# zgspose/PAVENet

Hardware: AMD Instinct MI355X
Metric: clips/sec (T=7, 800x1344) fwd (higher is better)
Workload: dtype f32 (exact 3-term bf16 split on the bf16 MFMA)

## Files before the change

### include/pave_hip.h

```cpp
#ifndef PAVE_HIP_H_
#define PAVE_HIP_H_

#include <stdint.h>

#ifdef __cplusplus
extern "C" {
#endif

#define PAVE_OK 0
#define PAVE_E_ARG (-1)
#define PAVE_E_LAUNCH (-2)
#define PAVE_E_STEP (-3)
#define PAVE_E_UNSUPPORTED (-4)

#define PAVE_ABI_VERSION 21
int pave_abi_version(void);
const char* pave_last_error(void);

int pave_ms_deform_attn_forward_f32(const float* value, const int64_t* spatial_shapes,
                                    const int64_t* level_start, const float* sampling_loc,
                                    const float* attn_weight, float* out, int bs, int S, int M,
                                    int D, int L, int Lq, int P, int im2col_step, void* stream);
int pave_ms_deform_attn_forward_f64(const double* value, const int64_t* spatial_shapes,
                                    const int64_t* level_start, const double* sampling_loc,
// ... 342 lines not shown
typedef struct pave_reid_plan {
  pave_reid_describe_plan d;
  const int32_t* ids[PAVE_TRACK_MAX_FRAMES];
  int32_t*       out_ids[PAVE_TRACK_MAX_FRAMES];
  int32_t*       out_sim[PAVE_TRACK_MAX_FRAMES];
  int            camera[PAVE_TRACK_MAX_FRAMES];
  int32_t* person;
  int32_t* track;
  int32_t* last;
  int32_t* hits;
  int32_t* hist;
  int32_t* frame;
  int32_t* next;
  int32_t* dropped;
  int32_t* pairs;
  int cameras, S, max_lost, match_thr, min_hits, gain;
} pave_reid_plan;
int pave_reid_describe_nv12(const pave_reid_describe_plan* plan, void* stream);
int pave_reid_describe_bgr(const pave_reid_describe_plan* plan, void* stream);
int pave_reid_update_nv12(const pave_reid_plan* plan, void* stream);
int pave_reid_update_bgr(const pave_reid_plan* plan, void* stream);

int pave_conv3x3_nhwc_f32(const float* x, const float* w, const float* bias, float* y, int N,
                          int H, int W, int Cin, int Cout, int stride, int relu, void* stream);

int pave_rows_gemm_bias_res_act_f32(const float* a, const float* a_bias, const float* a2,
                                    const float* w, const float* bias, const float* residual,
                                    float* out, long long M, int K, int K2, int N, int relu,
                                    void* stream);

int pave_bias_relu_maxpool_nhwc_f32(const float* x, const float* bias, float* y, int N, int H,
                                    int W, int C, void* stream);

#define PAVE_PLANES_FP16 16
int pave_gemm_bf16x3_f32(const float* a, const float* a_bias, const void* w_planes,
                         const float* bias, const float* residual, float* out, long long M, int K,
                         int N, int relu, int nplanes, void* stream);

int pave_gemm_fp16_act_f32(const void* a, int a_is_f16, const void* w_plane, const float* bias,
                           const float* residual, const float* gamma, const float* beta, float eps, void* out,
                           int out_is_f16, long long M, int K, int N, int relu, void* stream);

int pave_gemm_bf16x3_ex_f32(const float* a, const float* a_bias, const void* w_planes,
                            const float* bias, const float* residual, long long residual_rows,
                            float* out, float* out2, int n_split, long long M, int K, int N,
                            int relu, int nplanes, void* stream);

int pave_ref_update_f32(const float* tmp, const float* ref, float* out, long long n, float eps,
                        void* stream);

int pave_groupnorm_nhwc_f32(const float* x, const float* gamma, const float* beta, float* y,
                            long long y_batch_stride, int N, int HW, int C, int G, float eps,
                            double* partial, int nchunks, float* ab, void* stream);

typedef struct pave_gn_level {
  const float* x;
  const float* gamma;
  const float* beta;
  float* y;
  long long y_batch_stride;
  int HW;
  int nchunks;
  float eps;
} pave_gn_level;
int pave_groupnorm_levels_nhwc_f32(const pave_gn_level* levels, int nlev, int N, int C, int G, double* partial,
                                   float* ab, void* stream);
// ... 26 lines not shown
                                long long workspace_bytes, void* stream);

int pave_set_form_policy(int policy);
int pave_get_form_policy(void);

#define PAVE_FORM_ROWS 0
#define PAVE_FORM_ROWS_SPLITK 1
#define PAVE_FORM_ROWS_TILE 2
#define PAVE_FORM_LN 3
#define PAVE_FORM_CONV3X3 4
#define PAVE_FORM_CONV1X1S 5
#define PAVE_FORM_ENCPROJ 6
#define PAVE_ORDER_TILE 0
#define PAVE_ORDER_KSPLIT 1
#define PAVE_ORDER_SPLITK 2
#define PAVE_ORDER_TILE_LNPASS 3
#define PAVE_ORDER_KSPLIT_LNPASS 4
#define PAVE_ORDER_TILE_LN8 5
int pave_form_plan(long long M, int K, int N, int kind, int nplanes, int policy, int* order, int* ksplit);

int pave_bottleneck_chain_f32(const float* c1, const void* w2_planes, const float* b2, float* c2,
                              const void* w3_planes, const float* b3, const float* residual,
                              const float* a2, int k2, float* out, const void* w1n_planes,
                              const float* b1n, float* c1n, int cn, int N, int H, int W, int nplanes,
                              void* stream);

int pave_conv1x1_strided_split_f32(const float* x, const void* w_planes, const float* bias, float* y,
                                   int N, int H, int W, int Cin, int Cout, int stride, int relu,
                                   int nplanes, void* stream);

int pave_conv7x7s2_nchw_split_f32(const float* x, const void* w_planes, const float* bias, float* y,
                                  int N, int H, int W, int row_pitch, int Cout, int relu, int nplanes,
                                  void* stream);

int pave_repitch_rows_f32(const float* src, float* dst, long long rows, int W, int pitch, void* stream);

int pave_swin_window_attn_f32(const float* qkv, const float* bias_t, const float* pad_qkv, float* out, int B,
                              int H, int W, int C, int heads, int window, int shift, float scale, void* stream);

int pave_merge_softmax_partials_f32(const float* parts, float* out, int G, int U, int C, int H, void* stream);

int pave_split_bf16x3_f32(const float* x, void* planes, long long n, int nplanes, void* stream);

#define PAVE_AUG_MAX_AUGS 16
#define PAVE_AUG_MAX_SLOTS 128
#define PAVE_AUG_MAX_K 64
typedef struct pave_aug_plan {
  const float* bboxes[PAVE_AUG_MAX_AUGS];
  const float* kpts[PAVE_AUG_MAX_AUGS];
  const int32_t* keep[PAVE_AUG_MAX_AUGS];
  int32_t flip[PAVE_AUG_MAX_AUGS];
  float img_w[PAVE_AUG_MAX_SLOTS];
  float scale_factor[PAVE_AUG_MAX_SLOTS][4];
  int32_t flip_perm[PAVE_AUG_MAX_K];
  int32_t n_aug, B, N, K;
} pave_aug_plan;
int pave_aug_merge_nms_f32(const pave_aug_plan* plan, float score_thr, int max_num, int method, float iou_thr,
                           float sigma, float min_score, int offset, float* dets, int64_t* labels, float* kpts,
                           int64_t* inds, int32_t* keep, int32_t* count, void* stream);

int pave_hflip_canvas_f32(const float* x, float* y, const int32_t* valid_w, int valid_w_all, int n, int C, int Hp,
                          int Wp, void* stream);

#ifdef __cplusplus
}
#endif
// ... 2 lines not shown
```

### pavenet_amd/backbones.py

```python
import torch
import torch.nn as nn
import torch.nn.functional as F

from .bricks import BaseModule, build_norm_layer
from .registry import MMDET_MODELS


class BasicBlock(nn.Module):
    expansion = 1

    def __init__(self, inplanes, planes, stride=1, dilation=1, downsample=None, style='pytorch',
                 norm_cfg=dict(type='BN')):
        super().__init__()
        self.conv1 = nn.Conv2d(inplanes, planes, 3, stride, dilation, dilation, bias=False)
        self.bn1 = build_norm_layer(norm_cfg, planes)[1]
        self.conv2 = nn.Conv2d(planes, planes, 3, 1, 1, bias=False)
        self.bn2 = build_norm_layer(norm_cfg, planes)[1]
        self.relu = nn.ReLU(inplace=True)
        self.downsample = downsample
        self.pairs = (('conv1', 'bn1', True), ('conv2', 'bn2', False))


class Bottleneck(nn.Module):
    expansion = 4
# ... 50 lines not shown
        self.norm_eval = norm_eval
        self.style = style
        block, stage_blocks = self.arch_settings[depth]
        stage_blocks = stage_blocks[:num_stages]
        self.conv1 = nn.Conv2d(in_channels, stem_channels, 7, 2, 3, bias=False)
        self.bn1 = build_norm_layer(norm_cfg, stem_channels)[1]
        self.relu = nn.ReLU(inplace=True)
        self.maxpool = nn.MaxPool2d(kernel_size=3, stride=2, padding=1)
        self.res_layers = []
        inplanes = stem_channels
        for i, nb in enumerate(stage_blocks):
            planes = base_channels * 2**i
            layers = []
            for b in range(nb):
                stride = strides[i] if b == 0 else 1
                downsample = None
                if b == 0 and (stride != 1 or inplanes != planes * block.expansion):
                    downsample = nn.Sequential(
                        nn.Conv2d(inplanes, planes * block.expansion, 1, stride, bias=False),
                        build_norm_layer(norm_cfg, planes * block.expansion)[1])
                layers.append(block(inplanes, planes, stride, dilations[i], downsample, style,
                                    norm_cfg))
                inplanes = planes * block.expansion
            name = f'layer{i + 1}'
            self.add_module(name, nn.Sequential(*layers))
            self.res_layers.append(name)
        self.feat_dim = inplanes
        self._folded = None
        self.channels_last = True
        self.fused_tail_max_k = 256
        self.fused_ds_max_k = 128
        self.chain_stage64 = True
        self.chain_mode = 'full'
        self.deterministic_conv3x3 = False

    def init_weights(self):
        for m in self.modules():
            if isinstance(m, nn.Conv2d):
                nn.init.kaiming_normal_(m.weight, mode='fan_out', nonlinearity='relu')
            elif isinstance(m, (nn.BatchNorm2d, nn.GroupNorm)):
                nn.init.constant_(m.weight, 1)
                nn.init.constant_(m.bias, 0)
        for m in self.modules():
            if isinstance(m, Bottleneck):
                nn.init.constant_(m.bn3.weight, 0)
            elif isinstance(m, BasicBlock):
                nn.init.constant_(m.bn2.weight, 0)
        self._is_init = True

    def _params_key(self):
        from .bricks import SourceKey, module_tensors
        return SourceKey(module_tensors(self))

    def _stem_folded(self):
        from .bricks import SourceKey
        bn = self.bn1
        key = SourceKey([self.conv1.weight, bn.weight, bn.bias, bn.running_mean, bn.running_var])
        hit = self.__dict__.get('_stem_cache')
        if hit is None or hit[0] != key:
            mf = torch.channels_last if self.channels_last else torch.contiguous_format
            with torch.no_grad():
                hit = (key, tuple(t.contiguous(memory_format=mf) if t.dim() == 4 else t
                                  for t in _fold(self.conv1, self.bn1)))
            self.__dict__['_stem_cache'] = hit
        return hit[1]

    def _build_folded(self):
        key = self._params_key()
        if self._folded is not None and self._folded[0] == key:
            return self._folded[1]
        mf = torch.channels_last if self.channels_last else torch.contiguous_format
        with torch.no_grad():
            f = {'stem': tuple(t.contiguous(memory_format=mf) if t.dim() == 4 else t
                               for t in _fold(self.conv1, self.bn1))}
            for name in self.res_layers:
                for bi, blk in enumerate(getattr(self, name)):
                    for cn, bn, _ in blk.pairs:
                        w, b = _fold(getattr(blk, cn), getattr(blk, bn))
                        f[(name, bi, cn)] = (w.contiguous(memory_format=mf), b)
                        if cn == 'conv2' and w.shape[2:] == (3, 3) and w.shape[1] % 32 == 0 \
                                and w.shape[0] % 64 == 0:
                            f[(name, bi, 'conv2_taps')] = w.permute(2, 3, 1, 0).contiguous()
                        if cn == 'conv3' and w.shape[1] <= self.fused_tail_max_k \
                                and w.shape[1] % 32 == 0:
                            f[(name, bi, 'conv3_kn')] = w.flatten(1).t().contiguous()
                    if blk.downsample is not None:
                        w, b = _fold(blk.downsample[0], blk.downsample[1])
                        f[(name, bi, 'ds')] = (w.contiguous(memory_format=mf), b)
                        w3_kn = f.get((name, bi, 'conv3_kn'))
                        if w3_kn is not None and w.shape[1] % 32 == 0 and \
                                w3_kn.shape[0] + w.shape[1] <= self.fused_ds_max_k:
                            f[(name, bi, 'tail_ds_kn')] = (
                                torch.cat([w3_kn, w.flatten(1).t()], 0).contiguous(),
                                f[(name, bi, 'conv3')][1] + b)
        self._folded = (key, f)
        return f

    @staticmethod
    def _stem_split(x_nchw, w):
        from . import ops
        from .bricks import _split_cached, fused_mode, get_gemm_mode
        if not fused_mode() or torch.is_grad_enabled() or not x_nchw.is_cuda \
                or x_nchw.dtype != torch.float32 or tuple(w.shape) != (64, 3, 7, 7) \
                or x_nchw.shape[1] != 3 or x_nchw.shape[3] < 8 or not x_nchw.is_contiguous():
            return None
        wp = _split_cached(w, 'stem7x7', lambda planes: ops.split_stem7x7_weight(w.detach(), planes))
        if x_nchw.shape[3] % 4 or x_nchw.data_ptr() % 16:
            return ops.conv7x7s2_nchw_split(ops.repitch_rows(x_nchw), wp, valid_w=x_nchw.shape[3])
        return ops.conv7x7s2_nchw_split(x_nchw, wp)

    @staticmethod
    def _ds_bias(f, name, bi):
        key = (name, bi, 'ds_b3')
        if key not in f:
            f[key] = f[(name, bi, 'ds')][1] + f[(name, bi, 'conv3')][1]
        return f[key]

    @staticmethod
    def _as_rows(x):
        n, c, h, w = x.shape
        return x.permute(0, 2, 3, 1).reshape(-1, c), (n, h, w)

    @staticmethod
    def _as_map(rows, nhw):
        n, h, w = nhw
        return rows.view(n, h, w, rows.shape[-1]).permute(0, 3, 1, 2)

    def _stage64_chain_ok(self, name, x, f):
        from .bricks import _GEMM, fused_mode
        blocks = list(getattr(self, name))
        if blocks[0].downsample is not None and (name, 0, 'tail_ds_kn') not in f:
            return False
        if not (self.chain_stage64 and fused_mode() and not torch.is_grad_enabled()
                and x.is_contiguous(memory_format=torch.channels_last)
                and x.shape[0] * x.shape[2] * x.shape[3] >= _GEMM['min_rows']
                and all(isinstance(b, Bottleneck) for b in blocks)):
            return False
        for bi, blk in enumerate(blocks):
            c1, c2, c3 = blk.conv1, blk.conv2, blk.conv3
            if not (c1.out_channels == 64 and c1.stride == (1, 1)
                    and tuple(c2.weight.shape) == (64, 64, 3, 3) and c2.stride == (1, 1)
                    and c2.dilation == (1, 1) and c2.padding == (1, 1) and c2.groups == 1
# ... 122 lines not shown
                                      inplace_residual=True, a_bias=b2)
                else:
                    out = ops.rows_gemm_bias_res_act(yrows, w3_kn, None, idt, relu=True, out=idt,
                                                     a_bias=b2)
            else:
                idt = torch.addmm(bd + b3, xrows, wd.flatten(1).t())
                if w3_kn is not None:
                    out = ops.rows_gemm_bias_res_act(yrows, w3_kn, None, idt, relu=True, out=idt,
                                                     a_bias=b2)
                else:
                    out = torch.addmm(idt, yrows, w3.flatten(1).t())
                    ops.bias_act_rows_(out, None, None, relu=True)
        elif split3:
            out = linear_rows(yrows, w3.flatten(1), b3, relu=True, residual=rows,
                              inplace_residual=inplace_identity, a_bias=b2)
        elif w3_kn is not None:
            out = ops.rows_gemm_bias_res_act(yrows, w3_kn, b3, rows, relu=True,
                                             out=rows if inplace_identity else None, a_bias=b2)
        elif inplace_identity:
            out = rows.addmm_(yrows, w3.flatten(1).t())
            ops.bias_act_rows_(out, b3, None, relu=True)
        else:
            out = torch.addmm(rows, yrows, w3.flatten(1).t())
            ops.bias_act_rows_(out, b3, None, relu=True)
        return self._as_map(out, onhw)

    def forward(self, x):
        if self.input_type == 'mul_frames' and x.dim() == 5:
            x = x.flatten(0, 1)
        assert not self.training, 'pavenet_amd.ResNet is an inference (frozen BN) backbone'
        gemm_path = (self.channels_last and x.is_cuda and x.dtype == torch.float32
                     and self.style == 'pytorch')
        w, b = self._stem_folded()
        y = self._stem_split(x, w) if gemm_path else None
        if y is None and self.channels_last:
            x = x.contiguous(memory_format=torch.channels_last)
        if gemm_path:
            from . import ops
            if y is None:
                y = F.conv2d(x, w, None, 2, 3)
            x = ops.bias_relu_maxpool_nhwc(y, b)
        else:
            x = self.maxpool(F.relu_(F.conv2d(x, w, b, 2, 3)))
        f = self._build_folded()
        outs = []
        pre_c1 = None
        for i, name in enumerate(self.res_layers):
            if gemm_path and self._stage64_chain_ok(name, x, f):
                nxt = None
                if i + 1 < len(self.res_layers):
                    nb = getattr(self, self.res_layers[i + 1])[0]
                    if isinstance(nb, Bottleneck) and nb.conv1.stride == (1, 1) and \
                            nb.conv1.in_channels == 256 and nb.conv1.out_channels in (64, 128):
                        nxt = f[(self.res_layers[i + 1], 0, 'conv1')]
                x, pre_c1 = self._stage64_chain(name, x, f, nxt)
                if i in self.out_indices:
                    outs.append(x)
                continue
            for bi, blk in enumerate(getattr(self, name)):
                if gemm_path and isinstance(blk, Bottleneck):
                    x = self._bottleneck_gemm(blk, x, f, name, bi, inplace_identity=bi > 0,
                                              c1=pre_c1)
                    pre_c1 = None
                    continue
                identity = x
                y = x
                for cn, _, act in blk.pairs:
                    conv = getattr(blk, cn)
                    w, b = f[(name, bi, cn)]
                    y = F.conv2d(y, w, b, conv.stride, conv.padding, conv.dilation)
# ... 347 lines not shown
```

### pavenet_amd/csrc/pave_gemm_dma.hip

```cpp
#include <hip/hip_runtime.h>
#include <type_traits>
#include <stdint.h>

#include "pave_hip.h"
#include "pave_internal.h"
#include "pave_enc_math.h"

namespace {

typedef __bf16 bf16x8 __attribute__((ext_vector_type(8)));
typedef float f32x16 __attribute__((ext_vector_type(16)));
typedef unsigned u32x4 __attribute__((ext_vector_type(4)));
typedef float f32x4 __attribute__((ext_vector_type(4)));

constexpr int QBM = 128;
constexpr int QNS = 3;
constexpr int QCST = 36;

struct QConv {
  int H, W, Cin, Ho, Wo, stride;
  unsigned rcp;
};
struct QOut {
  float* out2;
// ... 1011 lines not shown
}

template <int PL>
__global__ __launch_bounds__(512) __attribute__((amdgpu_waves_per_eu(2, 2))) void gemm_q_ln_kernel(
    const float* __restrict__ A, const uint16_t* __restrict__ Wp, const float* __restrict__ bias,
    const float* residual, float* out, const int M, const int K, const int N, const QLn ln) {
  PAVE_CLOCK_BEGIN(5);
  gemm_q_body<4, 2, 0, false, true, false, 0, 1, PL>(A, Wp, bias, residual, out, M, K, N, 0, nullptr,
                                                     QConv{0, 0, 0, 0, 0, 0}, QOut{nullptr, 0, 0, N, 0}, ln);
  PAVE_CLOCK_END();
}

template <int PL, int IO = 0>
__global__ __launch_bounds__(256) __attribute__((amdgpu_waves_per_eu(2, 2))) void gemm_w_ln_kernel(
    const float* __restrict__ A, const uint16_t* __restrict__ Wp, const float* __restrict__ bias,
    const float* residual, float* out, const int M, const int K, const int N, const QLn ln) {
  PAVE_CLOCK_BEGIN(6);
  gemm_q_body<8, 1, 0, false, true, true, 0, 1, PL, false, IO>(A, Wp, bias, residual, out, M, K, N, 0, nullptr,
                                                               QConv{0, 0, 0, 0, 0, 0}, QOut{nullptr, 0, 0, N, 0}, ln);
  PAVE_CLOCK_END();
}

constexpr int SBM = 96;
constexpr int SWC = 50;
constexpr int SNSLAB = 11;

template <int R>
struct StemRows {
  static constexpr int WPC = 2 * R + 5;
  static constexpr int ROWS = 3 * WPC + 1;
  static constexpr int WIN = ((ROWS * SWC + 63) / 64) * 1024;
};

template <int R, int PL = 3>
__global__ __launch_bounds__(192) void stem7x7_qr_kernel(
    const float* __restrict__ x, const uint16_t* __restrict__ Wp, const float* __restrict__ bias,
    float* __restrict__ y, const int H, const int W, const int Ho, const int Wo, const int relu) {
  extern __shared__ __attribute__((aligned(1024))) unsigned char smem[];
  PAVE_CLOCK_BEGIN(7);
  const int tid = threadIdx.x, lane = tid & 63;
  const int wave = __builtin_amdgcn_readfirstlane(tid >> 6);
  const int lr = lane & 31, kh = lane >> 5;
  const int segs = (Wo + SBM - 1) / SBM;
  constexpr int WPC = StemRows<R>::WPC, ZROW = 3 * WPC;
  const int Hp = (Ho + R - 1) / R;
  const int seg = blockIdx.x % segs;
  const int oy = R * ((blockIdx.x / segs) % Hp);
  const int n = blockIdx.x / (segs * Hp);
  const int ox0 = seg * SBM;
  const int xs = 2 * ox0 - 4;
  const unsigned lds0 = (unsigned)(size_t)(__attribute__((address_space(3))) unsigned char*)smem;

  constexpr int NCH = StemRows<R>::ROWS * SWC;
  constexpr int NINS = StemRows<R>::WIN / 1024;
#pragma unroll
  for (int q = 0; q < (NINS + 2) / 3; ++q) {
    const int ins = wave + 3 * q;
    if (ins < NINS) {
      const int ci = ins * 64 + lane;
      const int row = ci / SWC, cc = ci - row * SWC;
      const int c = row / WPC, wy = row - WPC * c;
      const int iy = 2 * oy - 3 + wy, ix = xs + 4 * cc;
      const bool ok = ci < NCH && row < ZROW && iy >= 0 && iy < H && ix >= 0 && ix + 4 <= W;
      const float* src = ok ? x + (((long long)n * 3 + c) * H + iy) * W + ix
                            : reinterpret_cast<const float*>(g_zero_chunk);
      dma16_flat(src, lds0 + ins * 1024);
    }
  }
  const uint16_t* wl = Wp + ((long long)lr * 16 + kh * 8);
  u32x4 wf[2][PL][2];
// ... 28 lines not shown
#pragma unroll
    for (int j = 0; j < 2; ++j)
#pragma unroll
      for (int i = 0; i < 16; ++i) acc[r][j][i] = 0.f;
  asm volatile("s_waitcnt vmcnt(0)\n\ts_barrier" ::: "memory");
#pragma unroll
  for (int s = 0; s < SNSLAB; ++s) {
    const int cur = s & 1, nxt = cur ^ 1;
    if (s + 1 < SNSLAB) load_w(s + 1, nxt);
#pragma unroll
    for (int r = 0; r < R; ++r) {
      read_split(s, r);
      if constexpr (PL == 1) {
#pragma unroll
        for (int j = 0; j < 2; ++j)
          acc[r][j] = __builtin_amdgcn_mfma_f32_32x32x16_f16(
              __builtin_bit_cast(f16x8, apl[r][0]), __builtin_bit_cast(f16x8, wf[cur][0][j]), acc[r][j], 0, 0, 0);
      } else {
#pragma unroll
      for (int o = 2; o >= 0; --o)
#pragma unroll
        for (int pa = 0; pa <= o; ++pa)
#pragma unroll
          for (int j = 0; j < 2; ++j)
            acc[r][j] = __builtin_amdgcn_mfma_f32_32x32x16_bf16(
                __builtin_bit_cast(bf16x8, apl[r][pa]), __builtin_bit_cast(bf16x8, wf[cur][o - pa][j]),
                acc[r][j], 0, 0, 0);
      }
    }
  }
  asm volatile("s_waitcnt lgkmcnt(0)\n\ts_barrier" ::: "memory");
  float* Cs = reinterpret_cast<float*>(smem) + wave * 32 * QCST;
  const int erow = lane >> 3, ec4 = lane & 7;
#pragma unroll
  for (int r = 0; r < R; ++r) {
    float* const orow = y + ((long long)n * Ho + oy + r) * Wo * 64;
#pragma unroll
    for (int j = 0; j < 2; ++j) {
      const int col = j * 32 + ec4 * 4;
      const float4 b4 = bias ? *reinterpret_cast<const float4*>(bias + col) : make_float4(0.f, 0.f, 0.f, 0.f);
#pragma unroll
      for (int i = 0; i < 16; ++i) Cs[((i & 3) + 8 * (i >> 2) + 4 * kh) * QCST + lr] = acc[r][j][i];
      __builtin_amdgcn_fence(__ATOMIC_RELEASE, "wavefront");
      __builtin_amdgcn_wave_barrier();
      __builtin_amdgcn_fence(__ATOMIC_ACQUIRE, "wavefront");
#pragma unroll
      for (int ps = 0; ps < 4; ++ps) {
        const int lrow = ps * 8 + erow;
        const int ox = ox0 + wave * 32 + lrow;
        float4 v = *reinterpret_cast<const float4*>(Cs + lrow * QCST + ec4 * 4);
        v.x += b4.x, v.y += b4.y, v.z += b4.z, v.w += b4.w;
        if (relu) {
          v.x = fmaxf(v.x, 0.f), v.y = fmaxf(v.y, 0.f), v.z = fmaxf(v.z, 0.f), v.w = fmaxf(v.w, 0.f);
        }
        if (ox < Wo && oy + r < Ho) *reinterpret_cast<float4*>(orow + (long long)ox * 64 + col) = v;
      }
      __builtin_amdgcn_fence(__ATOMIC_RELEASE, "wavefront");
      __builtin_amdgcn_wave_barrier();
    }
  }
  PAVE_CLOCK_END();
}

template <int TN, int KIND, bool ABIAS, int RM = 1, int PL = 3, bool HT = false>
int launch_q(const float* a, const uint16_t* w, const float* bias, const float* residual, float* out,
             long long M, int K, int N, int relu, const float* a_bias, hipStream_t st, const QConv g,
// ... 784 lines not shown
             ? PAVE_OK : PAVE_E_LAUNCH;
}
extern "C" int pave_diag_clock_read(unsigned long long* out16) {
  if (!out16) return PAVE_E_ARG;
  if (hipDeviceSynchronize() != hipSuccess) return PAVE_E_LAUNCH;
  return hipMemcpyFromSymbol(out16, HIP_SYMBOL(g_clock_acc), 16 * sizeof(unsigned long long)) == hipSuccess
             ? PAVE_OK : PAVE_E_LAUNCH;
}
#endif

extern "C" int pave_bottleneck_chain_f32(const float* c1, const void* w2_planes, const float* b2, float* c2,
                                         const void* w3_planes, const float* b3, const float* residual,
                                         const float* a2, int k2, float* out, const void* w1n_planes,
                                         const float* b1n, float* c1n, int cn, int N, int H, int W,
                                         int nplanes, void* stream) {
  return pave_with_planes(q_planes(nplanes), "bottleneck_chain: nplanes must be 3 or PAVE_PLANES_FP16", [&](auto pl) {
    return bottleneck_chain_go<decltype(pl)::value>(c1, w2_planes, b2, c2, w3_planes, b3, residual, a2, k2, out,
                                                    w1n_planes, b1n, c1n, cn, N, H, W, stream);
  });
}

int pave_internal_stem7x7_q(const float* x, const void* w_stem, const float* bias, float* y, int N,
                            int H, int W, int pitch, int relu, void* stream, int planes) {
  const int Ho = (H - 1) / 2 + 1, Wo = (W - 1) / 2 + 1;
  const long long gx = (long long)N * Ho * ((Wo + SBM - 1) / SBM);
  if (gx >= (1ll << 31)) return pave_internal_fail(PAVE_E_ARG, "stem7x7: grid too large");
#ifndef PAVE_STEM_ROWS
#define PAVE_STEM_ROWS 2
#endif
  constexpr int R = PAVE_STEM_ROWS;
  const long long g2 = (long long)N * ((Ho + R - 1) / R) * ((Wo + SBM - 1) / SBM);
  hipStream_t st = reinterpret_cast<hipStream_t>(stream);
  const uint16_t* w = static_cast<const uint16_t*>(w_stem);
  if (planes == 1)
    return pave_launch<stem7x7_qr_kernel<R, 1>>(dim3((unsigned)g2), dim3(192), StemRows<R>::WIN, st, x, w, bias, y, H,
                                                pitch, Ho, Wo, relu);
  return pave_launch<stem7x7_qr_kernel<R, 3>>(dim3((unsigned)g2), dim3(192), StemRows<R>::WIN, st, x, w, bias, y, H,
                                              pitch, Ho, Wo, relu);
}
```

### pavenet_amd/csrc/pave_gemm_split.hip

```cpp
#include <hip/hip_runtime.h>
#include <stdint.h>

#include "pave_hip.h"
#include "pave_internal.h"

namespace {

typedef __bf16 bf16x8 __attribute__((ext_vector_type(8)));
typedef float f32x16 __attribute__((ext_vector_type(16)));
typedef unsigned u32x4 __attribute__((ext_vector_type(4)));
typedef float f32x4 __attribute__((ext_vector_type(4)));
typedef float f32x4_u __attribute__((ext_vector_type(4), aligned(4)));

constexpr int BK = 16;
constexpr int RST = 48;

__device__ __forceinline__ int stage_row_perm(int r) {
  return (r & ~7) | ((r & 3) << 1) | ((r >> 2) & 1);
}

__device__ __forceinline__ unsigned hi16(float x) { return __float_as_uint(x) & 0xffff0000u; }
__device__ __forceinline__ unsigned pack_hi(unsigned lo, unsigned hi) {
  return __builtin_amdgcn_perm(hi, lo, 0x07060302u);
}
// ... 750 lines not shown
  if (rc != PAVE_OK) return rc;
  return pave_internal_splitk_reduce(ws, parts, M, Cout, bias, residual, relu, y, stream);
}

int pave_conv1x1_strided_split_f32(const float* x, const void* w_planes, const float* bias, float* y,
                                   int N, int H, int W, int Cin, int Cout, int stride, int relu,
                                   int nplanes, void* stream) {
  if (!x || !w_planes || !y) return pave_internal_fail(PAVE_E_ARG, "conv1x1_strided_split: null pointer");
  if (N <= 0 || H <= 0 || W <= 0 || stride < 1 || stride > 4)
    return pave_internal_fail(PAVE_E_ARG, "conv1x1_strided_split: bad sizes (1 <= stride <= 4)");
  if (Cin % 64 != 0 || Cout % 128 != 0 || Cin <= 0 || Cout <= 0)
    return pave_internal_fail(PAVE_E_ARG, "conv1x1_strided_split: Cin %% 64 == 0 and Cout %% 128 == 0 required");
  const int Ho = (H - 1) / stride + 1, Wo = (W - 1) / stride + 1;
  const long long M = (long long)N * Ho * Wo;
  if (M >= (1ll << 31) || (long long)N * H * W * Cin >= (1ll << 40))
    return pave_internal_fail(PAVE_E_ARG, "conv1x1_strided_split: tensor too large");
  if (!q_planes(nplanes)) return pave_internal_fail(PAVE_E_ARG, "conv1x1_strided_split: nplanes must be 3 or PAVE_PLANES_FP16");
  if ((g_diag_variant != PAVE_DV_FIRST_GEN || nplanes != 3) && (long long)N * H * W * Cin * 4 < (1ll << 32)) {
    GemmQ q = gemm_q_call(x, w_planes, bias, nullptr, y, M, Cin, Cout, relu, nplanes, stream);
    q.rows = GEMMQ_CONV1X1S, q.H = H, q.W = W, q.Cin = Cin, q.Ho = Ho, q.Wo = Wo, q.stride = stride;
    return pave_internal_gemm_q(q);
  }
  if (nplanes != 3) return pave_internal_fail(PAVE_E_UNSUPPORTED, "conv1x1_strided_split: fp16 operands need a map below 4 GiB");
  const ConvGeom g{H, W, Cin, Ho, Wo, stride};
  return launch_gemm<2, 2, false, 3, false, 0, true>(x, static_cast<const uint16_t*>(w_planes), bias,
                                                     nullptr, y, M, Cin, Cout, relu, nullptr,
                                                     reinterpret_cast<hipStream_t>(stream), g);
}

int pave_conv7x7s2_nchw_split_f32(const float* x, const void* w_planes, const float* bias, float* y,
                                  int N, int H, int W, int row_pitch, int Cout, int relu, int nplanes,
                                  void* stream) {
  if (!x || !w_planes || !y) return pave_internal_fail(PAVE_E_ARG, "conv7x7s2_nchw_split: null pointer");
  if (N <= 0 || H <= 0 || W < 8 || (relu != 0 && relu != 1))
    return pave_internal_fail(PAVE_E_ARG, "conv7x7s2_nchw_split: bad sizes (W >= 8; relu 0 | 1)");
  if (row_pitch == 0) row_pitch = W;
  if (row_pitch < W || (row_pitch != W && ((row_pitch & 3) || (reinterpret_cast<uintptr_t>(x) & 15))))
    return pave_internal_fail(PAVE_E_ARG, "conv7x7s2_nchw_split: row_pitch >= W; a pitch beyond W must be a "
                                          "multiple of 4 on a 16-byte aligned image (pave_repitch_rows_f32)");
  if (Cout != 64)
    return pave_internal_fail(PAVE_E_UNSUPPORTED, "conv7x7s2_nchw_split: Cout == 64 (the ResNet / HRNet stem)");
  const int Ho = (H - 1) / 2 + 1, Wo = (W - 1) / 2 + 1;
  const long long M = (long long)N * Ho * Wo;
  if (M >= (1ll << 31) || (long long)N * 3 * H * row_pitch >= (1ll << 40))
    return pave_internal_fail(PAVE_E_ARG, "conv7x7s2_nchw_split: tensor too large");
  if (!q_planes(nplanes)) return pave_internal_fail(PAVE_E_ARG, "conv7x7s2_nchw_split: nplanes must be 3 or PAVE_PLANES_FP16");
  if ((g_diag_variant != PAVE_DV_FIRST_GEN || nplanes != 3 || row_pitch != W) && row_pitch % 4 == 0 &&
      (reinterpret_cast<uintptr_t>(x) & 15) == 0)
    return pave_internal_stem7x7_q(x, static_cast<const uint16_t*>(w_planes) + 12 * q_planes(nplanes) * 64 * 16, bias, y,
                                   N, H, W, row_pitch, relu, stream, q_planes(nplanes));
  if (nplanes != 3)
    return pave_internal_fail(PAVE_E_UNSUPPORTED, "conv7x7s2_nchw_split: fp16 operands need W %% 4 == 0 (or a repitched image) and a 16-byte aligned image");
  const ConvGeom g{H, W, 3, Ho, Wo, 2};
  return launch_gemm<2, 1, false, 3, false, 2, true>(x, static_cast<const uint16_t*>(w_planes), bias,
                                                     nullptr, y, M, 192, Cout, relu, nullptr,
                                                     reinterpret_cast<hipStream_t>(stream), g);
}

}
```

### pavenet_amd/csrc/pave_kernels.hip

```cpp
#include <hip/hip_runtime.h>
#include <stdint.h>
#include <stdio.h>
#include <stdlib.h>
#include <string.h>

#include "pave_hip.h"
#include "pave_internal.h"

namespace {

constexpr int kWave = 64;
constexpr int kHeads = 8;
constexpr int kDim = 32;
constexpr int kRowFloats = kHeads * kDim;
constexpr int kMaxLevels = 8;

thread_local char g_err[256] = "";

int fail(int code, const char* msg) {
  snprintf(g_err, sizeof(g_err), "%s", msg);
  return code;
}

template <typename scalar_t>
// ... 1191 lines not shown
  for (long long i = (long long)blockIdx.x * 256 + threadIdx.x; i < total;
       i += (long long)gridDim.x * 256) {
    const int c = (int)(i % c4) * 4;
    const long long pix = i / c4;
    const int ox = (int)(pix % Wo);
    const int oy = (int)((pix / Wo) % Ho);
    const long long n = pix / ((long long)Wo * Ho);
    float4 m = make_float4(-INFINITY, -INFINITY, -INFINITY, -INFINITY);
#pragma unroll
    for (int ky = 0; ky < 3; ++ky) {
      const int iy = oy * 2 - 1 + ky;
      if (iy < 0 || iy >= H) continue;
#pragma unroll
      for (int kx = 0; kx < 3; ++kx) {
        const int ix = ox * 2 - 1 + kx;
        if (ix < 0 || ix >= W) continue;
        const float4 v =
            *reinterpret_cast<const float4*>(x + ((n * H + iy) * W + ix) * C + c);
        m.x = fmaxf(m.x, v.x);
        m.y = fmaxf(m.y, v.y);
        m.z = fmaxf(m.z, v.z);
        m.w = fmaxf(m.w, v.w);
      }
    }
    const float4 b = *reinterpret_cast<const float4*>(bias + c);
    m.x = fmaxf(m.x + b.x, 0.f);
    m.y = fmaxf(m.y + b.y, 0.f);
    m.z = fmaxf(m.z + b.z, 0.f);
    m.w = fmaxf(m.w + b.w, 0.f);
    *reinterpret_cast<float4*>(y + pix * C + c) = m;
  }
}

__global__ __launch_bounds__(256) void groupnorm_stats_kernel(
    const float* __restrict__ x, double* __restrict__ partial, const int HW, const int C,
    const int G, const int nchunks) {
  __shared__ double sh[256][2];
  const int tpr = C >> 2;
  const int rpp = 256 / tpr;
  const int c4 = threadIdx.x % tpr, r0 = threadIdx.x / tpr;
  const int n = blockIdx.y, chunk = blockIdx.x;
  const int rows_per_chunk = (HW + nchunks - 1) / nchunks;
  const int rbeg = chunk * rows_per_chunk;
  const int rend = min(HW, rbeg + rows_per_chunk);
  const float* xb = x + (long long)n * HW * C + c4 * 4;
  double s = 0.0, q = 0.0;
  if (r0 < rpp)
    for (int r = rbeg + r0; r < rend; r += rpp) {
      const float4 v = *reinterpret_cast<const float4*>(xb + (long long)r * C);
      s += (double)((v.x + v.y) + (v.z + v.w));
      q += (double)((v.x * v.x + v.y * v.y) + (v.z * v.z + v.w * v.w));
    }
  sh[threadIdx.x][0] = (r0 < rpp) ? s : 0.0;
  sh[threadIdx.x][1] = (r0 < rpp) ? q : 0.0;
  __syncthreads();
  if (threadIdx.x < G) {
    const int tpg = (C / G) >> 2;
    double ts = 0.0, tq = 0.0;
    for (int r = 0; r < rpp; ++r)
      for (int j = 0; j < tpg; ++j) {
        const int t = r * tpr + threadIdx.x * tpg + j;
        ts += sh[t][0];
        tq += sh[t][1];
      }
    double* o = partial + (((long long)n * nchunks + chunk) * G + threadIdx.x) * 2;
    o[0] = ts;
// ... 522 lines not shown
int pave_rows_gemm_bias_res_act_f32(const float* a, const float* a_bias, const float* a2,
                                    const float* w, const float* bias, const float* residual,
                                    float* out, long long M, int K, int K2, int Nc, int relu,
                                    void* stream) {
  if (!a || !w || !out) return fail(PAVE_E_ARG, "rows_gemm: null pointer");
  if (M <= 0 || K <= 0 || K2 < 0 || Nc <= 0 || M >= (1ll << 31))
    return fail(PAVE_E_ARG, "rows_gemm: bad sizes (0 < M < 2^31)");
  if ((K2 > 0) != (a2 != nullptr)) return fail(PAVE_E_ARG, "rows_gemm: a2 and K2 go together");
  if (K % 32 != 0 || K2 % 32 != 0 || Nc % 64 != 0)
    return fail(PAVE_E_ARG, "rows_gemm: K, K2 %% 32 == 0 and N %% 64 == 0 required");
  const int bn = Nc % 128 == 0 ? 128 : 64;
  const long long gx = ((M + 127) / 128) * (Nc / bn);
  if (gx >= (1ll << 31)) return fail(PAVE_E_ARG, "rows_gemm: grid too large");
  hipStream_t st = reinterpret_cast<hipStream_t>(stream);
  if (bn == 128)
    return pave_launch<conv_nhwc_kernel<128, 1>>(dim3((unsigned)gx), dim3(256), 0, st, a, w, bias, residual, out, 1, 1,
                                                 (int)M, K, Nc, 1, (int)M, 1, relu, a_bias, a2, K2);
  return pave_launch<conv_nhwc_kernel<64, 1>>(dim3((unsigned)gx), dim3(256), 0, st, a, w, bias, residual, out, 1, 1,
                                              (int)M, K, Nc, 1, (int)M, 1, relu, a_bias, a2, K2);
}

int pave_bias_relu_maxpool_nhwc_f32(const float* x, const float* bias, float* y, int N, int H,
                                    int W, int C, void* stream) {
  if (!x || !bias || !y) return fail(PAVE_E_ARG, "bias_relu_maxpool: null pointer");
  if (N <= 0 || H <= 0 || W <= 0 || C <= 0 || C % 4 != 0)
    return fail(PAVE_E_ARG, "bias_relu_maxpool: bad sizes (C %% 4 == 0)");
  const int Ho = (H + 2 - 3) / 2 + 1, Wo = (W + 2 - 3) / 2 + 1;
  const long long total = (long long)N * Ho * Wo * (C / 4);
  const long long nb = std::min<long long>((total + 255) / 256, 256 * 64);
  return pave_launch<bias_relu_maxpool_kernel>(
      dim3((unsigned)nb), dim3(256), 0, reinterpret_cast<hipStream_t>(stream), x, bias, y, N, H, W, C, Ho, Wo);
}

int pave_groupnorm_nhwc_f32(const float* x, const float* gamma, const float* beta, float* y,
                            long long y_batch_stride, int N, int HW, int C, int G, float eps,
                            double* partial, int nchunks, float* ab, void* stream) {
  if (!x || !gamma || !beta || !y || !partial || !ab)
    return fail(PAVE_E_ARG, "groupnorm_nhwc: null pointer");
  if (N <= 0 || HW <= 0 || C <= 0 || G <= 0 || nchunks <= 0 || nchunks > 65535 || N > 65535)
    return fail(PAVE_E_ARG, "groupnorm_nhwc: sizes must be positive (N, nchunks <= 65535)");
  if (C % 4 != 0 || C > 1024 || C % G != 0 || (C / G) % 4 != 0 || G > 256 || 256 % (C / 4) != 0)
    return fail(PAVE_E_UNSUPPORTED,
                "groupnorm_nhwc: C %% 4 == 0, (C / G) %% 4 == 0, C / 4 divides 256, G <= 256");
  if (y_batch_stride < (long long)HW * C)
    return fail(PAVE_E_ARG, "groupnorm_nhwc: y_batch_stride smaller than one image");
  hipStream_t st = reinterpret_cast<hipStream_t>(stream);
  int rc = pave_launch<groupnorm_stats_kernel>(dim3((unsigned)nchunks, (unsigned)N), dim3(256), 0, st, x, partial, HW, C,
                                               G, nchunks);
  if (rc != PAVE_OK) return rc;
  rc = pave_launch<groupnorm_finalize_kernel>(dim3((unsigned)N), dim3(256), 0, st, partial, gamma, beta, ab, HW, C, G,
                                              nchunks, eps);
  if (rc != PAVE_OK) return rc;
  const long long total = (long long)N * HW * (C / 4);
  const long long nb = std::min<long long>((total + 255) / 256, 256 * 32);
  return pave_launch<groupnorm_apply_kernel>(dim3((unsigned)nb), dim3(256), 0, st, x, ab, y, y_batch_stride, N, HW, C);
}

int pave_groupnorm_levels_nhwc_f32(const pave_gn_level* levels, int nlev, int N, int C, int G, double* partial,
                                   float* ab, void* stream) {
  if (!levels || !partial || !ab) return fail(PAVE_E_ARG, "groupnorm_levels: null pointer");
  if (nlev <= 0 || nlev > 4) return fail(PAVE_E_ARG, "groupnorm_levels: 1 .. 4 levels per call");
  if (N <= 0 || N > 65535 || C <= 0 || G <= 0)
    return fail(PAVE_E_ARG, "groupnorm_levels: sizes must be positive (N <= 65535)");
  if (C % 4 != 0 || C > 1024 || C % G != 0 || (C / G) % 4 != 0 || G > 256 || 256 % (C / 4) != 0)
    return fail(PAVE_E_UNSUPPORTED,
                "groupnorm_levels: C %% 4 == 0, (C / G) %% 4 == 0, C / 4 divides 256, G <= 256");
// ... 55 lines not shown
```

### pavenet_amd/ops.py

```python
import contextlib
import ctypes
import numbers

import torch

from . import native


KERNEL_EVENTS = None
KERNEL_EVENT_TAGS = ('enc_tile', 'enc_grid_T1')
KERNEL_EVENT_SHAPES = None


def _stream_ptr():
    return torch.cuda.current_stream().cuda_stream


FORM_ROWS, FORM_ROWS_SPLITK, FORM_ROWS_TILE, FORM_LN, FORM_CONV3X3, FORM_CONV1X1S, FORM_ENCPROJ = (
    native.DEFINES['PAVE_FORM_' + n] for n in ('ROWS', 'ROWS_SPLITK', 'ROWS_TILE', 'LN', 'CONV3X3', 'CONV1X1S',
                                               'ENCPROJ'))
ORDER_TILE, ORDER_KSPLIT, ORDER_SPLITK, ORDER_TILE_LNPASS, ORDER_KSPLIT_LNPASS, ORDER_TILE_LN8 = (
    native.DEFINES['PAVE_ORDER_' + n] for n in ('TILE', 'KSPLIT', 'SPLITK', 'TILE_LNPASS', 'KSPLIT_LNPASS',
                                                'TILE_LN8'))

# ... 1605 lines not shown


def repitch_rows(x):
    _dev(x, 'x', torch.float32)
    W = x.shape[-1]
    pitch = (W + 3) // 4 * 4
    out = torch.empty(tuple(x.shape[:-1]) + (pitch,), dtype=torch.float32, device=x.device)
    rows = x.numel() // W
    _launch('pave_repitch_rows_f32', 'repitch_rows', x.device, x.data_ptr(), out.data_ptr(), rows, W, pitch)
    return out


def conv7x7s2_nchw_split(x, w_planes, bias=None, relu=False, valid_w=None):
    _dev(x, 'x', torch.float32)
    npl = _planes(w_planes, only=_Q_PLANES)
    _require(x.dim() == 4 and x.shape[1] == 3, 'conv7x7s2_nchw_split: x [N, 3, H, W] (NCHW, dense)')
    _require(w_planes.shape[0] == 23, 'conv7x7s2_nchw_split: w_planes from split_stem7x7_weight')
    N, _, H, pitch = x.shape
    W = pitch if valid_w is None else int(valid_w)
    _require(0 < W <= pitch and (W == pitch or pitch % 4 == 0), 'conv7x7s2_nchw_split: valid_w <= W, W % 4 == 0')
    Cout = w_planes.shape[2]
    if bias is not None:
        _dev(bias, 'bias', torch.float32)
        _require(bias.numel() == Cout, 'conv7x7s2_nchw_split: bias [Cout]')
    Ho, Wo = (H - 1) // 2 + 1, (W - 1) // 2 + 1
    y = torch.empty((N, Ho, Wo, Cout), dtype=torch.float32, device=x.device)
    _launch('pave_conv7x7s2_nchw_split_f32', 'conv7x7s2_nchw_split', x.device,
            x.data_ptr(), w_planes.data_ptr(), _ptr(bias),
            y.data_ptr(), N, H, W, pitch, Cout, int(bool(relu)), npl,
            tag='conv7x7_stem', flops=2 * N * Ho * Wo * Cout * 147, shape=(N * Ho * Wo, 147, Cout))
    return y.permute(0, 3, 1, 2)


def ref_update(tmp, ref, eps=1e-5):
    _require(tmp.is_cuda and tmp.dtype == torch.float32 and ref.dtype == torch.float32
             and tuple(tmp.shape) == tuple(ref.shape), 'ref_update: fp32 device tensors, same shape')
    if (tmp.dim() >= 2 and not tmp.is_contiguous() and tmp.stride(-1) == 1 and ref.is_contiguous()
            and tmp.numel() > 0 and tmp.stride(-2) >= tmp.shape[-1]
            and all(tmp.stride(i) == tmp.stride(i + 1) * tmp.shape[i + 1] for i in range(tmp.dim() - 2))):
        R, o = tmp.numel() // tmp.shape[-1], tmp.shape[-1]
        out = torch.empty_like(ref)
        _launch('pave_ref_update_frames_f32', 'ref_update', tmp.device, tmp.data_ptr(), ref.data_ptr(), out.data_ptr(),
                R, 1, tmp.stride(-2), o, R, float(eps), tag='ref_update')
        return out
    tmp, ref = tmp.contiguous(), ref.contiguous()
    out = torch.empty_like(tmp)
    if tmp.numel() == 0:
        return out
    _launch('pave_ref_update_f32', 'ref_update', tmp.device, tmp.data_ptr(), ref.data_ptr(), out.data_ptr(),
            tmp.numel(), float(eps), tag='ref_update')
    return out


def ref_update_frames(y, ref, T, o, group, eps=1e-5, out=None):
    _dev(y, 'y', torch.float32)
    _dev(ref, 'ref', torch.float32)
    R = y.shape[0]
    op = y.shape[1] // int(T)
    _require(y.dim() == 2 and op * T == y.shape[1] and op >= o and ref.shape[-1] == o
             and ref.numel() == R * T * o and R % int(group) == 0,
             'ref_update_frames: y [R, T*op], ref [R*T rows, o], R % group == 0')
    if out is None:
        out = torch.empty_like(ref)
    else:
        _dev(out, 'out', torch.float32)
        _require(tuple(out.shape) == tuple(ref.shape), 'ref_update_frames: out shaped like ref')
# ... 397 lines not shown
```

Before: 58.25.

## Fuse stem 7x7 conv with 3x3 maxpool via partial pooled outputs

Adds a pooled-partials epilogue to the stem 7x7 stride-2 conv kernel. It reduces each pair of conv output rows into horizontally pooled partial maxima plus tile-edge columns, and never writes the full 64-channel conv map. A small combine kernel then merges adjacent row pairs and tile edges, adds the bias and applies ReLU to produce the maxpooled output. This removes the write and re-read of the large full-resolution stem activation, at the cost of an extra launch and partial buffers. Max-before-bias is valid because the bias is per channel.

```diff
diff --git a/include/pave_hip.h b/include/pave_hip.h
--- a/include/pave_hip.h
+++ b/include/pave_hip.h
@@ -398,6 +398,9 @@
 int pave_bias_relu_maxpool_nhwc_f32(const float* x, const float* bias, float* y, int N, int H,
                                     int W, int C, void* stream);
 
+int pave_stem_pool_combine_f32(const float* pa, const float* pb, const float* pe, const float* bias, float* y,
+                               int N, int H, int W, void* stream);
+
 #define PAVE_PLANES_FP16 16
 int pave_gemm_bf16x3_f32(const float* a, const float* a_bias, const void* w_planes,
                          const float* bias, const float* residual, float* out, long long M, int K,
@@ -490,6 +493,9 @@
 int pave_conv7x7s2_nchw_split_f32(const float* x, const void* w_planes, const float* bias, float* y,
                                   int N, int H, int W, int row_pitch, int Cout, int relu, int nplanes,
                                   void* stream);
+
+int pave_conv7x7s2_pool_partials_f32(const float* x, const void* w_planes, float* pa, float* pb, float* pe,
+                                     int N, int H, int W, int row_pitch, int nplanes, void* stream);
 
 int pave_repitch_rows_f32(const float* src, float* dst, long long rows, int W, int pitch, void* stream);
 
diff --git a/pavenet_amd/backbones.py b/pavenet_amd/backbones.py
--- a/pavenet_amd/backbones.py
+++ b/pavenet_amd/backbones.py
@@ -106,6 +106,7 @@
         self.fused_ds_max_k = 128
         self.chain_stage64 = True
         self.chain_mode = 'full'
+        self.stem_pool_mode = 'fused'
         self.deterministic_conv3x3 = False
 
     def init_weights(self):
@@ -171,7 +172,7 @@
         return f
 
     @staticmethod
-    def _stem_split(x_nchw, w):
+    def _stem_split(x_nchw, w, pool_bias=None):
         from . import ops
         from .bricks import _split_cached, fused_mode, get_gemm_mode
         if not fused_mode() or torch.is_grad_enabled() or not x_nchw.is_cuda \
@@ -180,8 +181,13 @@
             return None
         wp = _split_cached(w, 'stem7x7', lambda planes: ops.split_stem7x7_weight(w.detach(), planes))
         if x_nchw.shape[3] % 4 or x_nchw.data_ptr() % 16:
-            return ops.conv7x7s2_nchw_split(ops.repitch_rows(x_nchw), wp, valid_w=x_nchw.shape[3])
-        return ops.conv7x7s2_nchw_split(x_nchw, wp)
+            x_nchw, valid_w = ops.repitch_rows(x_nchw), x_nchw.shape[3]
+        else:
+            valid_w = None
+        if pool_bias is not None:
+            pa, pb, pe, map_hw = ops.conv7x7s2_pool_partials(x_nchw, wp, valid_w=valid_w)
+            return ops.stem_pool_combine(pa, pb, pe, pool_bias, map_hw)
+        return ops.conv7x7s2_nchw_split(x_nchw, wp, valid_w=valid_w)
 
     @staticmethod
     def _ds_bias(f, name, bi):
@@ -370,10 +376,16 @@
         gemm_path = (self.channels_last and x.is_cuda and x.dtype == torch.float32
                      and self.style == 'pytorch')
         w, b = self._stem_folded()
-        y = self._stem_split(x, w) if gemm_path else None
+        assert self.stem_pool_mode in ('fused', 'separate'), self.stem_pool_mode
+        mp = self.maxpool
+        fuse_pool = (self.stem_pool_mode == 'fused' and (mp.kernel_size, mp.stride, mp.padding) == (3, 2, 1)
+                     and mp.dilation == 1 and not mp.ceil_mode)
+        y = self._stem_split(x, w, b if fuse_pool else None) if gemm_path else None
         if y is None and self.channels_last:
             x = x.contiguous(memory_format=torch.channels_last)
-        if gemm_path:
+        if gemm_path and y is not None and fuse_pool:
+            x = y
+        elif gemm_path:
             from . import ops
             if y is None:
                 y = F.conv2d(x, w, None, 2, 3)
diff --git a/pavenet_amd/csrc/pave_gemm_dma.hip b/pavenet_amd/csrc/pave_gemm_dma.hip
--- a/pavenet_amd/csrc/pave_gemm_dma.hip
+++ b/pavenet_amd/csrc/pave_gemm_dma.hip
@@ -1067,10 +1067,12 @@
   static constexpr int WIN = ((ROWS * SWC + 63) / 64) * 1024;
 };
 
-template <int R, int PL = 3>
+template <int R, int PL = 3, bool POOL = false>
 __global__ __launch_bounds__(192) void stem7x7_qr_kernel(
     const float* __restrict__ x, const uint16_t* __restrict__ Wp, const float* __restrict__ bias,
-    float* __restrict__ y, const int H, const int W, const int Ho, const int Wo, const int relu) {
+    float* __restrict__ y, const int H, const int W, const int Ho, const int Wo, const int relu,
+    float* __restrict__ pb, float* __restrict__ pe) {
+  static_assert(!POOL || R == 2, "the pooled-partials epilogue is that of one pool row pair per block");
   extern __shared__ __attribute__((aligned(1024))) unsigned char smem[];
   PAVE_CLOCK_BEGIN(7);
   const int tid = threadIdx.x, lane = tid & 63;
@@ -1165,6 +1167,47 @@
   asm volatile("s_waitcnt lgkmcnt(0)\n\ts_barrier" ::: "memory");
   float* Cs = reinterpret_cast<float*>(smem) + wave * 32 * QCST;
   const int erow = lane >> 3, ec4 = lane & 7;
+  if constexpr (POOL) {
+    const bool row1 = oy + 1 < Ho;
+    const int xw0 = ox0 + wave * 32;
+    const int Wq = (Wo + 1) >> 1, G = (Wo + 31) >> 5;
+    const long long pair = (long long)n * Hp + (oy >> 1);
+    float* const edge = pe + (pair * G + (xw0 >> 5)) * 128;
+#pragma unroll
+    for (int j = 0; j < 2; ++j) {
+#pragma unroll
+      for (int t = 0; t < 2; ++t) {
+#pragma unroll
+        for (int i = 0; i < 16; ++i) {
+          const float lo = row1 ? acc[1][j][i] : -INFINITY;
+          Cs[((i & 3) + 8 * (i >> 2) + 4 * kh) * QCST + lr] = t == 0 ? fmaxf(acc[0][j][i], lo) : lo;
+        }
+        __builtin_amdgcn_fence(__ATOMIC_RELEASE, "wavefront");
+        __builtin_amdgcn_wave_barrier();
+        __builtin_amdgcn_fence(__ATOMIC_ACQUIRE, "wavefront");
+        float* const prow = (t == 0 ? y : pb) + pair * Wq * 64 + j * 32 + ec4 * 4;
+#pragma unroll
+        for (int ps = 0; ps < 2; ++ps) {
+          const int q = ps * 8 + erow;
+          const int ox = xw0 + 2 * q;
+          const float* c = Cs + 2 * q * QCST + ec4 * 4;
+          float4 m = *reinterpret_cast<const float4*>(c);
+          const float4 hi = *reinterpret_cast<const float4*>(c + QCST);
+          if (q > 0) {
+            const float4 v = *reinterpret_cast<const float4*>(c - QCST);
+            m.x = fmaxf(m.x, v.x), m.y = fmaxf(m.y, v.y), m.z = fmaxf(m.z, v.z), m.w = fmaxf(m.w, v.w);
+          }
+          if (ox + 1 < Wo) m.x = fmaxf(m.x, hi.x), m.y = fmaxf(m.y, hi.y), m.z = fmaxf(m.z, hi.z), m.w = fmaxf(m.w, hi.w);
+          if (ox < Wo) *reinterpret_cast<float4*>(prow + (long long)(ox >> 1) * 64) = m;
+          if (ps == 1 && erow == 7 && ox + 1 < Wo) *reinterpret_cast<float4*>(edge + t * 64 + j * 32 + ec4 * 4) = hi;
+        }
+        __builtin_amdgcn_fence(__ATOMIC_RELEASE, "wavefront");
+        __builtin_amdgcn_wave_barrier();
+      }
+    }
+    PAVE_CLOCK_END();
+    return;
+  }
 #pragma unroll
   for (int r = 0; r < R; ++r) {
     float* const orow = y + ((long long)n * Ho + oy + r) * Wo * 64;
@@ -2015,9 +2058,36 @@
   const long long g2 = (long long)N * ((Ho + R - 1) / R) * ((Wo + SBM - 1) / SBM);
   hipStream_t st = reinterpret_cast<hipStream_t>(stream);
   const uint16_t* w = static_cast<const uint16_t*>(w_stem);
+  float* const none = nullptr;
   if (planes == 1)
     return pave_launch<stem7x7_qr_kernel<R, 1>>(dim3((unsigned)g2), dim3(192), StemRows<R>::WIN, st, x, w, bias, y, H,
-                                                pitch, Ho, Wo, relu);
+                                                pitch, Ho, Wo, relu, none, none);
   return pave_launch<stem7x7_qr_kernel<R, 3>>(dim3((unsigned)g2), dim3(192), StemRows<R>::WIN, st, x, w, bias, y, H,
-                                              pitch, Ho, Wo, relu);
-}
+                                              pitch, Ho, Wo, relu, none, none);
+}
+
+extern "C" int pave_conv7x7s2_pool_partials_f32(const float* x, const void* w_planes, float* pa, float* pb, float* pe,
+                                                int N, int H, int W, int row_pitch, int nplanes, void* stream) {
+  if (!x || !w_planes || !pa || !pb || !pe)
+    return pave_internal_fail(PAVE_E_ARG, "conv7x7s2_pool_partials: null pointer");
+  if (N <= 0 || H <= 0 || W <= 0) return pave_internal_fail(PAVE_E_ARG, "conv7x7s2_pool_partials: bad sizes");
+  if (row_pitch == 0) row_pitch = W;
+  if (row_pitch < W) return pave_internal_fail(PAVE_E_ARG, "conv7x7s2_pool_partials: row_pitch >= W");
+  if ((row_pitch & 3) || (reinterpret_cast<uintptr_t>(x) & 15))
+    return pave_internal_fail(PAVE_E_UNSUPPORTED, "conv7x7s2_pool_partials: row_pitch %% 4 == 0 on a 16-byte aligned "
+                                                  "image (pave_repitch_rows_f32)");
+  const int planes = q_planes(nplanes);
+  if (!planes) return pave_internal_fail(PAVE_E_ARG, "conv7x7s2_pool_partials: nplanes must be 3 or PAVE_PLANES_FP16");
+  const int Ho = (H - 1) / 2 + 1, Wo = (W - 1) / 2 + 1;
+  if ((long long)N * Ho * Wo >= (1ll << 31) || (long long)N * 3 * H * row_pitch >= (1ll << 40))
+    return pave_internal_fail(PAVE_E_ARG, "conv7x7s2_pool_partials: tensor too large");
+  const long long g2 = (long long)N * ((Ho + 1) / 2) * ((Wo + SBM - 1) / SBM);
+  hipStream_t st = reinterpret_cast<hipStream_t>(stream);
+  const uint16_t* w = static_cast<const uint16_t*>(w_planes) + 12 * planes * 64 * 16;
+  const float* const nobias = nullptr;
+  if (planes == 1)
+    return pave_launch<stem7x7_qr_kernel<2, 1, true>>(dim3((unsigned)g2), dim3(192), StemRows<2>::WIN, st, x, w, nobias,
+                                                      pa, H, row_pitch, Ho, Wo, 0, pb, pe);
+  return pave_launch<stem7x7_qr_kernel<2, 3, true>>(dim3((unsigned)g2), dim3(192), StemRows<2>::WIN, st, x, w, nobias,
+                                                    pa, H, row_pitch, Ho, Wo, 0, pb, pe);
+}
diff --git a/pavenet_amd/csrc/pave_gemm_split.hip b/pavenet_amd/csrc/pave_gemm_split.hip
--- a/pavenet_amd/csrc/pave_gemm_split.hip
+++ b/pavenet_amd/csrc/pave_gemm_split.hip
@@ -806,8 +806,8 @@
                                   int N, int H, int W, int row_pitch, int Cout, int relu, int nplanes,
                                   void* stream) {
   if (!x || !w_planes || !y) return pave_internal_fail(PAVE_E_ARG, "conv7x7s2_nchw_split: null pointer");
-  if (N <= 0 || H <= 0 || W < 8 || (relu != 0 && relu != 1))
-    return pave_internal_fail(PAVE_E_ARG, "conv7x7s2_nchw_split: bad sizes (W >= 8; relu 0 | 1)");
+  if (N <= 0 || H <= 0 || W <= 0 || (relu != 0 && relu != 1))
+    return pave_internal_fail(PAVE_E_ARG, "conv7x7s2_nchw_split: bad sizes (relu 0 | 1)");
   if (row_pitch == 0) row_pitch = W;
   if (row_pitch < W || (row_pitch != W && ((row_pitch & 3) || (reinterpret_cast<uintptr_t>(x) & 15))))
     return pave_internal_fail(PAVE_E_ARG, "conv7x7s2_nchw_split: row_pitch >= W; a pitch beyond W must be a "
@@ -825,6 +825,7 @@
                                    N, H, W, row_pitch, relu, stream, q_planes(nplanes));
   if (nplanes != 3)
     return pave_internal_fail(PAVE_E_UNSUPPORTED, "conv7x7s2_nchw_split: fp16 operands need W %% 4 == 0 (or a repitched image) and a 16-byte aligned image");
+  if (W < 8) return pave_internal_fail(PAVE_E_ARG, "conv7x7s2_nchw_split: W >= 8 (or a repitched image)");
   const ConvGeom g{H, W, 3, Ho, Wo, 2};
   return launch_gemm<2, 1, false, 3, false, 2, true>(x, static_cast<const uint16_t*>(w_planes), bias,
                                                      nullptr, y, M, 192, Cout, relu, nullptr,
diff --git a/pavenet_amd/csrc/pave_kernels.hip b/pavenet_amd/csrc/pave_kernels.hip
--- a/pavenet_amd/csrc/pave_kernels.hip
+++ b/pavenet_amd/csrc/pave_kernels.hip
@@ -1247,6 +1247,35 @@
   }
 }
 
+__global__ __launch_bounds__(256) void stem_pool_combine_kernel(
+    const float* __restrict__ pa, const float* __restrict__ pb, const float* __restrict__ pe,
+    const float* __restrict__ bias, float* __restrict__ y, const int Hq, const int Wq, const int G) {
+  const int c = (threadIdx.x & 15) * 4, px = threadIdx.x >> 4;
+  const int xq = blockIdx.x * 16 + px, j = blockIdx.y;
+  if (xq >= Wq) return;
+  const long long row = (long long)blockIdx.z * Hq + j;
+  const long long at = (row * Wq + xq) * 64 + c;
+  const bool has_edge = px == 0 && blockIdx.x > 0;
+  const long long et = (row * G + ((int)blockIdx.x - 1)) * 128 + c;
+  const float4 ninf = make_float4(-INFINITY, -INFINITY, -INFINITY, -INFINITY);
+  const float4 va = *reinterpret_cast<const float4*>(pa + at);
+  float4 vb = ninf, ea = ninf, eb = ninf;
+  if (j > 0) vb = *reinterpret_cast<const float4*>(pb + at - (long long)Wq * 64);
+  if (has_edge) ea = *reinterpret_cast<const float4*>(pe + et);
+  if (has_edge && j > 0) eb = *reinterpret_cast<const float4*>(pe + et - (long long)G * 128 + 64);
+  const float4 b = *reinterpret_cast<const float4*>(bias + c);
+  float4 m;
+  m.x = fmaxf(fmaxf(fmaxf(fmaxf(-INFINITY, va.x), vb.x), ea.x), eb.x);
+  m.y = fmaxf(fmaxf(fmaxf(fmaxf(-INFINITY, va.y), vb.y), ea.y), eb.y);
+  m.z = fmaxf(fmaxf(fmaxf(fmaxf(-INFINITY, va.z), vb.z), ea.z), eb.z);
+  m.w = fmaxf(fmaxf(fmaxf(fmaxf(-INFINITY, va.w), vb.w), ea.w), eb.w);
+  m.x = fmaxf(m.x + b.x, 0.f);
+  m.y = fmaxf(m.y + b.y, 0.f);
+  m.z = fmaxf(m.z + b.z, 0.f);
+  m.w = fmaxf(m.w + b.w, 0.f);
+  *reinterpret_cast<float4*>(y + at) = m;
+}
+
 __global__ __launch_bounds__(256) void groupnorm_stats_kernel(
     const float* __restrict__ x, double* __restrict__ partial, const int HW, const int C,
     const int G, const int nchunks) {
@@ -1835,6 +1864,16 @@
       dim3((unsigned)nb), dim3(256), 0, reinterpret_cast<hipStream_t>(stream), x, bias, y, N, H, W, C, Ho, Wo);
 }
 
+int pave_stem_pool_combine_f32(const float* pa, const float* pb, const float* pe, const float* bias, float* y,
+                               int N, int H, int W, void* stream) {
+  if (!pa || !pb || !pe || !bias || !y) return fail(PAVE_E_ARG, "stem_pool_combine: null pointer");
+  if (N <= 0 || H <= 0 || W <= 0) return fail(PAVE_E_ARG, "stem_pool_combine: bad sizes");
+  const int Hq = (H + 1) / 2, Wq = (W + 1) / 2, G = (W + 31) / 32;
+  if (N > 65535 || Hq > 65535) return fail(PAVE_E_ARG, "stem_pool_combine: N, (H + 1) / 2 <= 65535");
+  return pave_launch<stem_pool_combine_kernel>(dim3((unsigned)((Wq + 15) / 16), (unsigned)Hq, (unsigned)N), dim3(256), 0,
+                                               reinterpret_cast<hipStream_t>(stream), pa, pb, pe, bias, y, Hq, Wq, G);
+}
+
 int pave_groupnorm_nhwc_f32(const float* x, const float* gamma, const float* beta, float* y,
                             long long y_batch_stride, int N, int HW, int C, int G, float eps,
                             double* partial, int nchunks, float* ab, void* stream) {
diff --git a/pavenet_amd/ops.py b/pavenet_amd/ops.py
--- a/pavenet_amd/ops.py
+++ b/pavenet_amd/ops.py
@@ -1661,6 +1661,54 @@
     return y.permute(0, 3, 1, 2)
 
 
+def conv7x7s2_pool_partials(x, w_planes, valid_w=None, out=None):
+    _dev(x, 'x', torch.float32)
+    npl = _planes(w_planes, only=_Q_PLANES)
+    _require(x.dim() == 4 and x.shape[1] == 3, 'conv7x7s2_pool_partials: x [N, 3, H, W] (NCHW, dense)')
+    _require(w_planes.shape[0] == 23 and w_planes.shape[2] == 64,
+             'conv7x7s2_pool_partials: w_planes from split_stem7x7_weight, 64 channels')
+    N, _, H, pitch = x.shape
+    W = pitch if valid_w is None else int(valid_w)
+    _require(0 < W <= pitch and pitch % 4 == 0, 'conv7x7s2_pool_partials: valid_w <= W, W % 4 == 0')
+    Ho, Wo = (H - 1) // 2 + 1, (W - 1) // 2 + 1
+    Hq, Wq, G = (Ho + 1) // 2, (Wo + 1) // 2, (Wo + 31) // 32
+    if out is None:
+        pa = torch.empty((N, Hq, Wq, 64), dtype=torch.float32, device=x.device)
+        pb = torch.empty((N, Hq, Wq, 64), dtype=torch.float32, device=x.device)
+        pe = torch.empty((N, Hq, G, 2, 64), dtype=torch.float32, device=x.device)
+    else:
+        pa, pb, pe = out
+        for t, nm in ((pa, 'pa'), (pb, 'pb'), (pe, 'pe')):
+            _dev(t, nm, torch.float32)
+        _require(tuple(pa.shape) == (N, Hq, Wq, 64) and tuple(pb.shape) == (N, Hq, Wq, 64)
+                 and tuple(pe.shape) == (N, Hq, G, 2, 64),
+                 'conv7x7s2_pool_partials: out = (pa, pb [N, Hq, Wq, 64], pe [N, Hq, G, 2, 64])')
+    _launch('pave_conv7x7s2_pool_partials_f32', 'conv7x7s2_pool_partials', x.device,
+            x.data_ptr(), w_planes.data_ptr(), pa.data_ptr(), pb.data_ptr(), pe.data_ptr(), N, H, W, pitch, npl,
+            tag='conv7x7_stem', flops=2 * N * Ho * Wo * 64 * 147, shape=(N * Ho * Wo, 147, 64))
+    return pa, pb, pe, (Ho, Wo)
+
+
+def stem_pool_combine(pa, pb, pe, bias, map_hw, out=None):
+    Ho, Wo = map_hw
+    Hq, Wq, G = (Ho + 1) // 2, (Wo + 1) // 2, (Wo + 31) // 32
+    N = pa.shape[0]
+    for t, nm in ((pa, 'pa'), (pb, 'pb'), (pe, 'pe'), (bias, 'bias')):
+        _dev(t, nm, torch.float32)
+    _require(tuple(pa.shape) == (N, Hq, Wq, 64) and tuple(pb.shape) == (N, Hq, Wq, 64)
+             and tuple(pe.shape) == (N, Hq, G, 2, 64) and bias.numel() == 64,
+             'stem_pool_combine: pa, pb [N, Hq, Wq, 64], pe [N, Hq, G, 2, 64], bias [64]')
+    if out is None:
+        y = torch.empty((N, Hq, Wq, 64), dtype=torch.float32, device=pa.device)
+    else:
+        y = out
+        _dev(y, 'out', torch.float32)
+        _require(tuple(y.shape) == (N, Hq, Wq, 64), 'stem_pool_combine: out [N, Hq, Wq, 64]')
+    _launch('pave_stem_pool_combine_f32', 'stem_pool_combine', pa.device,
+            pa.data_ptr(), pb.data_ptr(), pe.data_ptr(), bias.data_ptr(), y.data_ptr(), N, Ho, Wo, tag='stem_pool')
+    return y.permute(0, 3, 1, 2)
+
+
 def ref_update(tmp, ref, eps=1e-5):
     _require(tmp.is_cuda and tmp.dtype == torch.float32 and ref.dtype == torch.float32
              and tuple(tmp.shape) == tuple(ref.shape), 'ref_update: fp32 device tensors, same shape')
```

Result: no change. 58.59, median of 6 (+0.6%).
